# yandooo/cilium

Measured on AMD Instinct MI355X. Metric: L7 verdicts/sec + scanned GB/s (HBM roofline frac), 1/2/4/8 MI355X, higher is better.
Workload: dtype u8

## Files before the change

cilium_amd/csrc/kernels/kafka_classify.hip:

```cpp
#include <hip/hip_runtime.h>

#include "../device_tables.h"
#include "kafka_dec.h"
#include "launch.h"

namespace l7 {

namespace {

constexpr int kBlock = 256;


__device__ __forceinline__ uint32_t le_load4(Cur &c, const uint8_t *p) {
    const uintptr_t a = (uintptr_t)p;
    const uint32_t k = (uint32_t)(a & 15);
    if (k <= 12) {
        cur_fill(c, a);
        const uint32_t w0 = c.w0, w1 = c.w1, w2 = c.w2, w3 = c.w3;
        const uint32_t i = k >> 2;
        const uint32_t lo = i == 0 ? w0 : i == 1 ? w1 : i == 2 ? w2 : w3;
        const uint32_t hi = i == 0 ? w1 : i == 1 ? w2 : i == 2 ? w3 : 0u;
        return __builtin_amdgcn_alignbyte(hi, lo, k & 3);
    }
    uint32_t v = 0;
    for (int i = 0; i < 4; i++) v |= cur_byte(c, p + i) << (8 * i);
    return v;
}
__device__ __forceinline__ uint32_t bswap(uint32_t x) { return __builtin_amdgcn_perm(0, x, 0x00010203u); }

struct GRd {
    static constexpr bool kWin = true;
    const uint8_t *b;
    uintptr_t lastc;
    Cur cur;
    uint8_t *stage;
    uint32_t hlim;
    __device__ __forceinline__ void stage_head() {
        crc_stage(stage, reinterpret_cast<const uint8_t *>((uintptr_t)b & ~(uintptr_t)15), lastc);
        hlim = 64 - (uint32_t)((uintptr_t)b & 15);
    }
    __device__ __forceinline__ uint32_t slot_le4(uint32_t rel) {
        asm volatile("" : "+v"(rel));
        const uint32_t la = (uint32_t)(uintptr_t)(stage + 16 * lane_id());
        const uint32_t w0 = rel >> 2, w1 = w0 < 15 ? w0 + 1 : 15;
        uint32_t lo, hi;
        asm volatile("s_waitcnt vmcnt(0)\n\tds_read_b32 %0, %2\n\tds_read_b32 %1, %3\n\ts_waitcnt lgkmcnt(0)"
                     : "=&v"(lo), "=&v"(hi)
                     : "v"(la + ((w0 >> 2) << 10) + ((w0 & 3) << 2)), "v"(la + ((w1 >> 2) << 10) + ((w1 & 3) << 2))
                     : "memory");
        return __builtin_amdgcn_alignbyte(hi, lo, rel & 3);
    }
    __device__ __forceinline__ uint32_t le4(uint32_t pos) {
        if (pos + 4 <= hlim) return slot_le4(pos + (uint32_t)((uintptr_t)b & 15));
        return le_load4(cur, b + pos);
    }
    __device__ __forceinline__ uint64_t be(uint32_t pos, int n) {
        if (n <= 4 && pos + 4 <= hlim) {
            const uint32_t v = bswap(slot_le4(pos + (uint32_t)((uintptr_t)b & 15)));
            return n == 4 ? v : v >> (32 - 8 * n);
        }
        return be_load(cur, b + pos, n);
    }
    __device__ __forceinline__ void win9(uint32_t pos, uint32_t (&x)[9]) {
        const uintptr_t a = (uintptr_t)(b + pos);
        const uintptr_t c0 = a & ~(uintptr_t)15;
        uint32_t w[16];
        {
            hlim = 0;
            crc_stage(stage, reinterpret_cast<const uint8_t *>(c0), lastc);
            const uint32_t la = (uint32_t)(uintptr_t)(stage + 16 * lane_id());
            uint4 v0, v1, v2, v3;
            asm volatile("s_waitcnt vmcnt(0)\n\t"
                         "ds_read_b128 %0, %4\n\tds_read_b128 %1, %4 offset:1024\n\t"
                         "ds_read_b128 %2, %4 offset:2048\n\tds_read_b128 %3, %4 offset:3072\n\t"
                         "s_waitcnt lgkmcnt(0)"
                         : "=v"(v0), "=v"(v1), "=v"(v2), "=v"(v3)
                         : "v"(la)
                         : "memory");
            const uint4 vv[4] = {v0, v1, v2, v3};
#pragma unroll
            for (int k = 0; k < 4; k++) {
                w[4 * k] = vv[k].x; w[4 * k + 1] = vv[k].y; w[4 * k + 2] = vv[k].z; w[4 * k + 3] = vv[k].w;
            }
        }
        const uint32_t s = (uint32_t)(a & 15), q = s >> 2;
#pragma unroll
        for (int i = 0; i < 9; i++) {
            const uint32_t lo = q == 0 ? w[i] : q == 1 ? w[i + 1] : q == 2 ? w[i + 2] : w[i + 3];
            const uint32_t hi = q == 0 ? w[i + 1] : q == 1 ? w[i + 2] : q == 2 ? w[i + 3] : w[i + 4];
            x[i] = __builtin_amdgcn_alignbyte(hi, lo, s & 3);
        }
        cur.line = c0 + 16 <= lastc ? c0 + 16 : ~(uintptr_t)0;
        cur.w0 = w[4]; cur.w1 = w[5]; cur.w2 = w[6]; cur.w3 = w[7];
    }
    __device__ __forceinline__ uint32_t win_be4(uint32_t rel) { return bswap(slot_le4(rel)); }
};

template <class R>
struct KD {
    R *r;
    uint32_t pos, end;
    int32_t limit;
    int err;
};
template <class R>
__device__ __forceinline__ uint32_t kd_read(KD<R> &d, uint32_t n) {
    const uint32_t at = d.pos;
    if (n == 0) return at;
    uint32_t a = d.end - d.pos;
    if (d.limit >= 0 && (uint32_t)d.limit < a) a = (uint32_t)d.limit;
    if (a == 0) { d.err = 1; return at; }
    const uint32_t take = a < n ? a : n;
    d.pos += take;
    if (d.limit >= 0) d.limit -= (int32_t)take;
    if (take < n) d.err = 2;
    return at;
}
template <class R>
__device__ __forceinline__ int64_t kd_int(KD<R> &d, int n) {
    if (d.err) return 0;
    const uint32_t at = kd_read(d, (uint32_t)n);
    if (d.err) return 0;
    const uint64_t v = d.r->be(at, n);
    return n == 1 ? (int64_t)(int8_t)v : n == 2 ? (int64_t)(int16_t)v : n == 4 ? (int64_t)(int32_t)v : (int64_t)v;
}
template <class R>
__device__ __forceinline__ void kd_skip(KD<R> &d, int n) {
    if (d.err) return;
    kd_read(d, (uint32_t)n);
}
template <class R>
__device__ __forceinline__ void kd_string(KD<R> &d, uint32_t &off, uint32_t &len) {
    off = 0; len = 0;
    if (d.err) return;
    const int16_t sl = (int16_t)kd_int(d, 2);
    if (d.err || sl < 1) return;
    const uint32_t at = kd_read(d, (uint32_t)sl);
    if (d.err) return;
    off = at; len = (uint32_t)sl;
}
template <class R>
__device__ __forceinline__ int32_t kd_arraylen(KD<R> &d, bool nullable, bool &bad) {
    const int32_t l = (int32_t)kd_int(d, 4);
    bad = false;
    if (l < 0) { if (nullable) return -1; bad = true; return 0; }
    if ((uint32_t)l > kMaxParseBuf) { bad = true; return 0; }
    return l;
}
template <class R>
__device__ __forceinline__ bool kd_bulk(KD<R> &d, int32_t np, uint32_t esize) {
    if (d.err || np < 0) return false;
    uint32_t a = d.end - d.pos;
    if (d.limit >= 0 && (uint32_t)d.limit < a) a = (uint32_t)d.limit;
    const uint64_t need = (uint64_t)(uint32_t)np * esize;
    if (need > a) return false;
    d.pos += (uint32_t)need;
    if (d.limit >= 0) d.limit -= (int32_t)need;
    return true;
}
template <class R>
__device__ __forceinline__ void kd_bytes(KD<R> &d) {
    if (d.err) return;
    const int32_t sl = (int32_t)kd_int(d, 4);
    if (d.err || sl < 1) return;
    if ((uint32_t)sl > kMaxParseBuf) { d.err = 3; return; }
    kd_read(d, (uint32_t)sl);
}

template <class R, class H>
__device__ __forceinline__ int kd_message_set(R &r, uint32_t &pos, uint32_t end, int32_t size, int16_t version,
                                              bool &zflag, H &h) {
    if (size < 0) return 0;
    if ((uint32_t)size > kMaxParseBuf) return -1;
    KD<R> dec{&r, pos, end, size, 0};
    int rc = 0;
    if constexpr (R::kWin) {
        const uint32_t hmin = version >= 1 ? 22u : 14u;
        for (;;) {
            uint32_t avail = dec.end - dec.pos;
            if ((uint32_t)dec.limit < avail) avail = (uint32_t)dec.limit;
            if (avail < 12 + hmin) break;
            uint32_t x[9];
            r.win9(dec.pos, x);
            const uint32_t msize = bswap(x[2]);
            if ((int32_t)msize < (int32_t)hmin || 12 + msize > avail) break;
            const uint32_t at = dec.pos + 12;
            const uint32_t crc = bswap(x[3]);
            const uint32_t attr = (x[4] >> 8) & 0xFF;
            const int32_t klen = (int32_t)bswap(version >= 1 ? __builtin_amdgcn_alignbyte(x[7], x[6], 2)
                                                             : __builtin_amdgcn_alignbyte(x[5], x[4], 2));
            const uint32_t ko = at + (version >= 1 ? 14u : 6u);
            uint32_t vo = ko + 4;
            int32_t vlen;
            if (klen < 1) {
                vlen = (int32_t)bswap(version >= 1 ? __builtin_amdgcn_alignbyte(x[8], x[7], 2)
                                                   : __builtin_amdgcn_alignbyte(x[6], x[5], 2));
            } else {
                if ((uint32_t)klen > msize || vo + (uint32_t)klen + 4 > at + msize) break;
                vo += (uint32_t)klen;
                const uint32_t rel = vo - dec.pos + (uint32_t)((uintptr_t)(r.b + dec.pos) & 15);
                if (rel + 4 <= 64) {
                    vlen = (int32_t)r.win_be4(rel);
                } else {
                    const Cur keep = r.cur;
                    vlen = (int32_t)r.be(vo, 4);
                    r.cur = keep;
                }
            }
            if (vlen >= 1 && ((uint32_t)vlen > msize || vo + 4 + (uint32_t)vlen > at + msize)) break;
            dec.pos = at + msize;
            dec.limit -= (int32_t)(12 + msize);
            if (!h.msg_win(at + 4, msize - 4, crc)) { pos = dec.pos; return 0; }
            if ((attr & 3) == 3) { pos = dec.pos; return 0; }
            if (attr & 3) zflag = true;
        }
    }
    for (;;) {
        kd_skip(dec, 8);
        if (dec.err) break;
        const int32_t msize = (int32_t)kd_int(dec, 4);
        if (dec.err || msize <= 0) break;
        if ((uint32_t)msize > kMaxParseBuf) { rc = -1; break; }
        const uint32_t at = kd_read(dec, (uint32_t)msize);
        if (dec.err) break;
        KD<R> md{&r, at, at + (uint32_t)msize, -1, 0};
        const uint32_t crc = (uint32_t)kd_int(md, 4);
        if (msize <= 4) break;
        if (!h.msg(at + 4, (uint32_t)msize - 4, crc)) break;
        kd_skip(md, 1);
        const int8_t attr = (int8_t)kd_int(md, 1);
        if (version >= 1) kd_skip(md, 8);
        const int codec = attr & 3;
        if (codec == 3) break;
        kd_bytes(md);
        kd_bytes(md);
        if (md.err) { rc = -1; break; }
        if (codec != 0) zflag = true;
    }
    pos = dec.pos;
    return rc;
}

__device__ __forceinline__ bool is_topic_api_key(int k) {
    if (k < 0 || k > 37) return false;
    const uint64_t m = (1ull << 0) | (1ull << 1) | (1ull << 2) | (1ull << 3) | (1ull << 4) | (1ull << 5) | (1ull << 6) |
                       (1ull << 8) | (1ull << 9) | (1ull << 19) | (1ull << 20) | (1ull << 21) | (1ull << 23) |
                       (1ull << 24) | (1ull << 27) | (1ull << 28) | (1ull << 34) | (1ull << 35) | (1ull << 37);
    return (m >> k) & 1;
}
__device__ __forceinline__ int kind_typed(int kind) {
    return (kind == 0 || kind == 1 || kind == 2 || kind == 3 || kind == 8 || kind == 9) ? 1 : (kind == 10 ? 2 : 0);
}

template <class R, class H>
__device__ __forceinline__ int kafka_walk(R &r, uint32_t rawlen, int kind, bool &zflag, H &h) {
    KD<R> d{&r, 0, rawlen, -1, 0};
    bool bad = false;
    int rc = 0;
    kd_skip(d, 4); kd_skip(d, 2);
    const int16_t ver = (int16_t)kd_int(d, 2);
    kd_skip(d, 4);
    uint32_t co, cl;
    kd_string(d, co, cl);
    if (!d.err && cl > 0) h.client(co, cl);
    int32_t nt, np;
    uint32_t o, l;
    switch (kind) {
    case 0:
        if (ver >= 3) kd_string(d, o, l);
        kd_skip(d, 2); kd_skip(d, 4);
        nt = kd_arraylen(d, false, bad);
        if (bad) { rc = -1; break; }
        for (int32_t t = 0; t < nt && rc == 0; t++) {
            kd_string(d, o, l);
            if (d.err) break;
            h.topic(o, l);
            np = kd_arraylen(d, false, bad);
            if (bad) { rc = -1; break; }
            for (int32_t p = 0; p < np; p++) {
                kd_skip(d, 4);
                if (d.err) { rc = -1; break; }
                const int32_t ss = (int32_t)kd_int(d, 4);
                if (d.err) { rc = -1; break; }
                rc = kd_message_set(r, d.pos, d.end, ss, ver, zflag, h);
                if (rc) break;
            }
        }
        break;
    case 1:
        kd_skip(d, 4); kd_skip(d, 4); kd_skip(d, 4);
        if (ver >= 3) kd_skip(d, 4);
        if (ver >= 4) kd_skip(d, 1);
        nt = kd_arraylen(d, false, bad);
        if (bad) { rc = -1; break; }
        for (int32_t t = 0; t < nt && !d.err; t++) {
            kd_string(d, o, l);
            h.topic(o, l);
            np = kd_arraylen(d, false, bad);
            if (bad) { rc = -1; break; }
            if (kd_bulk(d, np, ver >= 5 ? 24u : 16u)) continue;
            for (int32_t p = 0; p < np && !d.err; p++) {
                kd_skip(d, 4); kd_skip(d, 8);
                if (ver >= 5) kd_skip(d, 8);
                kd_skip(d, 4);
            }
        }
        break;
    case 2:
        kd_skip(d, 4);
        if (ver >= 2) kd_skip(d, 1);
        nt = kd_arraylen(d, false, bad);
        if (bad) { rc = -1; break; }
        for (int32_t t = 0; t < nt && !d.err; t++) {
            kd_string(d, o, l);
            h.topic(o, l);
            np = kd_arraylen(d, false, bad);
            if (bad) { rc = -1; break; }
            if (kd_bulk(d, np, ver == 0 ? 16u : 12u)) continue;
            for (int32_t p = 0; p < np && !d.err; p++) {
                kd_skip(d, 4); kd_skip(d, 8);
                if (ver == 0) kd_skip(d, 4);
            }
        }
        break;
    case 3:
        nt = kd_arraylen(d, true, bad);
        if (bad) { rc = -1; break; }
        for (int32_t t = 0; t < nt && !d.err; t++) {
            kd_string(d, o, l);
            if (!d.err) h.topic(o, l);
        }
        if (ver >= 4) kd_skip(d, 1);
        break;
    case 8:
        kd_string(d, o, l);
        if (ver >= 1) { kd_skip(d, 4); kd_string(d, o, l); }
        if (ver >= 2) kd_skip(d, 8);
        nt = kd_arraylen(d, false, bad);
        if (bad) { rc = -1; break; }
        for (int32_t t = 0; t < nt && !d.err; t++) {
            kd_string(d, o, l);
            h.topic(o, l);
            np = kd_arraylen(d, false, bad);
            if (bad) { rc = -1; break; }
            for (int32_t p = 0; p < np && !d.err; p++) {
                kd_skip(d, 4); kd_skip(d, 8);
                if (ver == 1) kd_skip(d, 8);
                uint32_t o2, l2;
                kd_string(d, o2, l2);
            }
        }
        break;
    case 9:
        kd_string(d, o, l);
        nt = kd_arraylen(d, true, bad);
        if (bad) { rc = -1; break; }
        for (int32_t t = 0; t < nt && !d.err; t++) {
            kd_string(d, o, l);
            h.topic(o, l);
            np = kd_arraylen(d, false, bad);
            if (bad) { rc = -1; break; }
            if (kd_bulk(d, np, 4u)) continue;
            for (int32_t p = 0; p < np && !d.err; p++) kd_skip(d, 4);
        }
        break;
    case 10:
        kd_string(d, o, l);
        if (ver >= 1) kd_skip(d, 1);
        break;
    }
    if (rc == 0 && d.err) rc = -1;
    return rc;
}

template <class R>
__device__ __forceinline__ int32_t str_lookup(const DevStrSlot *tab, uint32_t mask, const uint8_t *strings, R &r,
                                              uint32_t pos, uint32_t n) {
    uint32_t h = kWHashSeed;
    uint32_t p0 = 0, p1 = 0, p2 = 0, p3 = 0;
    for (uint32_t i = 0; i < n; i += 4) {
        const uint32_t rem = n - i;
        const uint32_t keep = rem >= 4 ? 0xFFFFFFFFu : (1u << (8 * rem)) - 1u;
        const uint32_t w = r.le4(pos + i) & keep;
        h = l7_whash_step(h, w);
        p0 = i == 0 ? w : p0;
        p1 = i == 4 ? w : p1;
        p2 = i == 8 ? w : p2;
        p3 = i == 12 ? w : p3;
    }
    h = l7_whash_final(h, n);
    for (uint32_t slot = h & mask;; slot = (slot + 1) & mask) {
        const DevStrSlot e = tab[slot];
        if (!e.used) return -1;
        if (e.hash == h && e.len == n) {
            bool eq = e.pre[0] == p0 && e.pre[1] == p1 && e.pre[2] == p2 && e.pre[3] == p3;
            const uint32_t *t = reinterpret_cast<const uint32_t *>(strings + e.str_off);
            for (uint32_t i = 16; i < n && eq; i += 4) {
                const uint32_t rem = n - i;
                const uint32_t keep = rem >= 4 ? 0xFFFFFFFFu : (1u << (8 * rem)) - 1u;
                eq = t[i >> 2] == (r.le4(pos + i) & keep);
            }
            if (eq) return e.id;
        }
    }
}

struct ReqInfo {
    uint32_t kv;
    int32_t client;
    __device__ __forceinline__ int kind_() const { return (int)(int16_t)(kv >> 16); }
    __device__ __forceinline__ int version_() const { return (int)(int16_t)(kv & 0xFFFF); }
    __device__ __forceinline__ int typed_() const { return kind_typed(kind_()); }
};

__device__ __forceinline__ bool rule_matches(const DevKafkaRule &r, const ReqInfo &q) {
    if (!r.any_key && (q.kind_() < 0 || q.kind_() > 63 || !((r.keymask >> q.kind_()) & 1))) return false;
    if (r.has_version && r.version != q.version_()) return false;
    if (!r.has_topic && r.client < 0) return true;
    if (q.typed_() == 1) return r.client < 0 || r.client == q.client;
    if (q.typed_() == 2) return true;
    return !(r.has_topic && is_topic_api_key(q.kind_()));
}

__device__ __forceinline__ uint32_t topic_first(const KafkaTables &T, const DevKafkaRuleset &rs, const ReqInfo &q,
                                                int32_t tid) {
    if (tid < 0 || rs.ntopics == 0) return kInf;
    uint32_t off, cnt;
    if (rs.tdense_off != ~0u) {
        const uint4 *ep = reinterpret_cast<const uint4 *>(T.index + rs.tdense_off +
                                                          (uint32_t)(sizeof(DevKafkaTopicEnt) / 4) * (uint32_t)tid);
        const uint4 e0 = ep[0], e1 = ep[1], e2 = ep[2];
        off = e0.y;
        cnt = e0.z;
        if (cnt == 0) return kInf;
        DevKafkaRule r0;
        const uint32_t w[6] = {e1.x, e1.y, e1.z, e1.w, e2.x, e2.y};
        __builtin_memcpy(&r0, w, sizeof r0);
        if (rule_matches(r0, q)) return e0.x;
        for (uint32_t i = 1; i < cnt; i++) {
            const uint32_t p = T.index[off + i];
            if (rule_matches(T.rules[rs.rule_first + p], q)) return p;
        }
        return kInf;
    } else {
        const uint32_t *dir = T.index + rs.topics_off;
        uint32_t lo = 0, hi = rs.ntopics;
        while (lo < hi) {
            const uint32_t m = (lo + hi) >> 1;
            if (dir[3 * m] < (uint32_t)tid) lo = m + 1; else hi = m;
        }
        if (lo >= rs.ntopics || dir[3 * lo] != (uint32_t)tid) return kInf;
        off = dir[3 * lo + 1];
        cnt = dir[3 * lo + 2];
    }
    for (uint32_t i = 0; i < cnt; i++) {
        const uint32_t p = T.index[off + i];
        if (rule_matches(T.rules[rs.rule_first + p], q)) return p;
    }
    return kInf;
}

__device__ __forceinline__ uint32_t matches_rule(const KafkaTables &T, const DevKafkaRuleset &rs, const ReqInfo &q,
                                                 uint32_t ntopics, uint32_t cmax) {
    uint32_t best = kInf;
    if (ntopics == 0) {
        const int key = (q.kind_() >= 0 && q.kind_() < 64) ? q.kind_() : 64;
        const uint32_t off = T.index[rs.bykey_off + 2 * key], cnt = T.index[rs.bykey_off + 2 * key + 1];
        for (uint32_t i = 0; i < cnt; i++) {
            const uint32_t p = T.index[off + i];
            if (rule_matches(T.rules[rs.rule_first + p], q)) { best = p; break; }
        }
    } else {
        for (uint32_t i = 0; i < rs.ntopicless; i++) {
            const uint32_t p = T.index[rs.topicless_off + i];
            if (p >= cmax) break;
            if (rule_matches(T.rules[rs.rule_first + p], q)) { best = p; break; }
        }
        if (best == kInf) best = cmax;
    }
    return best;
}

struct NoTopicLog {};
struct TopicLog {
    LogSpan *row;
    uint32_t stride;
};
template <class L>
struct ExactHooks {
    const KafkaTables &T;
    const DevKafkaRuleset &rs;
    ReqInfo &q;
    GRd &r;
    const uint32_t *crctab;
    uint8_t *stage;
    uint32_t ntopics, cmax;
    L log;
    __device__ __forceinline__ void client(uint32_t o, uint32_t l) {
        q.client = str_lookup(T.client_hash, T.client_mask, T.strings, r, o, l);
        if (q.client < 0) q.client = -2;
    }
    __device__ __forceinline__ void topic(uint32_t o, uint32_t l) {
        if (q.typed_() != 1) return;
        if constexpr (!std::is_same<L, NoTopicLog>::value) {
            if (ntopics < log.stride) log.row[ntopics] = LogSpan{o, l};
        }
        ntopics++;
        const int32_t tid = l > 0 ? str_lookup(T.topic_hash, T.topic_mask, T.strings, r, o, l) : -1;
        const uint32_t e = topic_first(T, rs, q, tid);
        cmax = cmax > e ? cmax : e;
    }
    __device__ __forceinline__ bool msg(uint32_t pos, uint32_t n, uint32_t stored) {
        r.hlim = 0;
        return crc32_ieee_staged(crctab, r.cur, r.b + pos, n, stage, r.lastc) == stored;
    }
    __device__ __forceinline__ bool msg_win(uint32_t pos, uint32_t n, uint32_t stored) {
        return crc32_ieee_window(crctab, r.cur, r.b + pos, n, stage, r.lastc) == stored;
    }
};

}

template <int kWaves, bool kLog>
__global__ __launch_bounds__(kBlock) __attribute__((amdgpu_waves_per_eu(kWaves, 8))) void kafka_classify_kernel(
    Batch B, KafkaTables T, const uint32_t *__restrict__ sel, const uint32_t *__restrict__ sel_count,
    uint32_t answer_other, uint32_t *__restrict__ zlist, uint32_t *__restrict__ zcount, uint32_t *__restrict__ work,
    uint32_t main_sweep, LogRec *__restrict__ lrec, LogSpan *__restrict__ ltopics, uint32_t lstride) {
    const uint32_t n = B.n, nconns = B.nconns;
    static_assert(kBlock >= 256, "one CRC table entry per thread");
    __shared__ uint32_t crctab[kCrcTables * 256];
    __shared__ __attribute__((aligned(16))) uint8_t crcstage[kBlock / 64][4096];
    uint8_t *stage = crcstage[__builtin_amdgcn_readfirstlane((int)(threadIdx.x >> 6))];
    crc_tables_init(crctab, threadIdx.x);
    constexpr int kCls = L7_KAFKA_CLASSES;
    uint32_t kc[kCls] = {n};
    uint32_t m = n;
    if (sel) {
        m = 0;
        for (int c = 0; c < kCls; c++) { kc[c] = sel_count[c]; m += kc[c]; }
    }
    const uint32_t stride = main_sweep ? main_sweep : gridDim.x * kBlock;
    auto next_entry = [&](uint32_t i) -> uint32_t {
        if (!work) return i + stride;
        const uint32_t lane = lane_id();
        uint32_t t = 0;
        if (lane == (uint32_t)__builtin_amdgcn_readfirstlane(lane)) t = atomicAdd(work, 64u);
        return stride + __builtin_amdgcn_readfirstlane(t) + lane;
    };
    for (uint32_t i = main_sweep ? next_entry(0) : blockIdx.x * kBlock + threadIdx.x; i < m; i = next_entry(i)) {
        uint32_t idx = i;
        if (sel) {
            uint32_t c = 0, j = i;
            bool hit = false;
#pragma unroll
            for (int k = kCls - 1; k > 0; k--) {
                if (!hit) {
                    if (j >= kc[k]) j -= kc[k];
                    else { c = (uint32_t)k; hit = true; }
                }
            }
            idx = sel[(size_t)c * n + j];
        }
        const uint32_t ci = B.conn_ids[idx];
        const DevConn conn = ci < nconns ? B.conns[ci] : DevConn{-1, PROTO_NONE, 0, 0xFFFF};
        const uint64_t off = B.offs[idx];
        const uint32_t len = B.lens[idx];
        uint8_t verdict = V_PARSE_ERROR;
        int32_t rule = -1;
        uint32_t consumed = 0;
        bool zflag = false;
        if (conn.proto != PROTO_KAFKA || conn.ruleset < 0 || (uint32_t)conn.ruleset >= T.nrulesets) {
            if (!answer_other || (L7_PROTO_OWNED(conn.proto) && conn.proto != PROTO_KAFKA)) continue;
            verdict = V_UNSUPPORTED;
        }
        do {
            if (verdict == V_UNSUPPORTED) break;
            if (!l7_in_arena(off, len, B.arena_len)) { verdict = V_UNSUPPORTED; break; }
            if (len < 4) { verdict = V_INCOMPLETE; break; }
            GRd r{B.arena + off, ((uintptr_t)(B.arena + off) + len - 1) & ~(uintptr_t)15, {}, stage, 0};
            r.stage_head();
            r.cur.line = ~(uintptr_t)0;
            const int32_t size = (int32_t)r.be(0, 4);
            if (size <= 0) break;
            if (len < 6) { verdict = V_INCOMPLETE; break; }
            if ((uint64_t)(uint32_t)size + 4 > kMaxParseBuf) break;
            const uint32_t rawlen = (uint32_t)size + 4;
            if (rawlen > len) { verdict = V_INCOMPLETE; break; }
            if (rawlen < 12) break;
            ReqInfo q;
            q.kv = (uint32_t)r.be(4, 4);
            q.client = -2;
            const DevKafkaRuleset &rs = T.rulesets[conn.ruleset];
            using Log = typename std::conditional<kLog, TopicLog, NoTopicLog>::type;
            Log lg{};
            if constexpr (kLog) lg = TopicLog{ltopics + (size_t)idx * lstride, lstride};
            ExactHooks<Log> h{T, rs, q, r, crctab, stage, 0, 0, lg};
            if (q.typed_() && kafka_walk(r, rawlen, q.kind_(), zflag, h) == -1) break;
            consumed = rawlen;
            verdict = V_DENY;
            if constexpr (kLog) {
                const uint32_t corr = (uint32_t)r.be(8, 4);
                uint4 *o = reinterpret_cast<uint4 *>(lrec + idx);
                o[0] = make_uint4(LOG_KAFKA | (h.ntopics > lstride ? 0x100u : 0u) | (q.kv & 0xFFFF0000u),
                                  q.kv & 0xFFFFu, corr, h.ntopics);
                o[1] = make_uint4(0, 0, 0, 0);
            }
            if (!rs.any) break;
            const uint32_t best = matches_rule(T, rs, q, h.ntopics, h.cmax);
            if (best != kInf) { verdict = V_ALLOW; rule = T.rules[rs.rule_first + best].gid; }
        } while (false);
        B.verdict[idx] = verdict;
        B.rule[idx] = rule;
        B.consumed[idx] = consumed;
        if (zflag && zlist && (verdict == V_ALLOW || verdict == V_DENY)) zlist[atomicAdd(zcount, 1u)] = idx;
    }
}

hipError_t KafkaPhaseTimes(uint64_t *, bool) { return hipErrorNotSupported; }

hipError_t LaunchKafkaClassify(const Batch &B, const KafkaTables &T, const uint32_t *sel, const uint32_t *sel_count,
                               bool answer_other, uint32_t *zlist, uint32_t *zcount, uint32_t *work,
                               hipStream_t stream, int leave_per_cu, bool helper, const LogOut *log) {
    if (B.n == 0) return hipSuccess;
    uint32_t blocks = (B.n + kBlock - 1) / kBlock;
    const bool beside = leave_per_cu > 0;
    if (helper && (!beside || !work)) return hipErrorInvalidValue;
    const bool lg = log != nullptr;
    const auto kernel = lg ? kafka_classify_kernel<4, true>
                           : (beside ? kafka_classify_kernel<6, false> : kafka_classify_kernel<5, false>);
    static int cus[2][2] = {}, per_cu[2][2] = {};
    if (cus[lg][beside] == 0) {
        int dev = 0, c = 0, p = 0;
        if (hipGetDevice(&dev) == hipSuccess &&
            hipDeviceGetAttribute(&c, hipDeviceAttributeMultiprocessorCount, dev) == hipSuccess &&
            hipOccupancyMaxActiveBlocksPerMultiprocessor(&p, kernel, kBlock, 0) == hipSuccess && c > 0 && p > 0) {
            per_cu[lg][beside] = p;
            cus[lg][beside] = c;
        } else {
            per_cu[lg][beside] = 32;
            cus[lg][beside] = 256;
        }
    }
    const int pc = per_cu[lg][beside], ncu = cus[lg][beside];
    const int slots = beside && pc > leave_per_cu ? pc - leave_per_cu : pc;
    if (!work) blocks = blocks > 8192 ? 8192 : blocks;
    else if (blocks > (uint32_t)(ncu * slots)) blocks = (uint32_t)(ncu * slots);
    const uint32_t grid = helper ? min(blocks, (uint32_t)(ncu * min(leave_per_cu, pc))) : blocks;
    const uint32_t main_sweep = helper ? blocks * (uint32_t)kBlock : 0u;
    LogRec *lrec = lg ? log->rec : nullptr;
    LogSpan *ltopics = lg ? log->topics : nullptr;
    hipLaunchKernelGGL(kernel, dim3(grid), dim3(kBlock), 0, stream, B, T, sel, sel_count, answer_other ? 1u : 0u, zlist,
                       zcount, work, main_sweep, lrec, ltopics, lg ? log->stride : 0u);
    return hipGetLastError();
}

}
```

cilium_amd/csrc/kernels/kafka_dec.h:

```cpp
#pragma once
#include <hip/hip_runtime.h>

#include <stdint.h>

#include "gmem.h"

namespace l7 {
namespace {

constexpr uint32_t kMaxParseBuf = 6553500;
constexpr int kCrcSlices = 8;
constexpr int kCrcTables = 8;
__device__ __forceinline__ void crc_tables_init(uint32_t *tab, uint32_t t) {
    if (t < 256) {
        uint32_t c = t;
        for (int k = 0; k < 8; k++) c = (c & 1) ? 0xEDB88320u ^ (c >> 1) : c >> 1;
        tab[t] = c;
    }
    __syncthreads();
    if (t < 256) {
        uint32_t v = tab[t];
        for (int k = 1; k < kCrcTables; k++) {
            v = (v >> 8) ^ tab[v & 0xFF];
            tab[k * 256 + t] = v;
        }
    }
    __syncthreads();
}
__device__ __forceinline__ uint32_t crc_slice8(const uint32_t *tab, uint32_t lo, uint32_t hi) {
    return tab[7 * 256 + (lo & 0xFF)] ^ tab[6 * 256 + ((lo >> 8) & 0xFF)] ^ tab[5 * 256 + ((lo >> 16) & 0xFF)] ^
           tab[4 * 256 + (lo >> 24)] ^ tab[3 * 256 + (hi & 0xFF)] ^ tab[2 * 256 + ((hi >> 8) & 0xFF)] ^
           tab[1 * 256 + ((hi >> 16) & 0xFF)] ^ tab[hi >> 24];
}
constexpr uint32_t kInf = 0xFFFFFFFFu;
__device__ __forceinline__ uint32_t lane_id() {
    return __builtin_amdgcn_mbcnt_hi(~0u, __builtin_amdgcn_mbcnt_lo(~0u, 0u));
}

struct Cur {
    uintptr_t line;
    uint32_t w0, w1, w2, w3;
};
__device__ __forceinline__ void cur_fill(Cur &c, uintptr_t a) {
    const uintptr_t ln = a & ~(uintptr_t)15;
    if (ln != c.line) {
        const uint4 v = gload16(ln);
        c.w0 = v.x; c.w1 = v.y; c.w2 = v.z; c.w3 = v.w;
        c.line = ln;
    }
}
__device__ __forceinline__ uint32_t cur_word(const Cur &c, uint32_t k) {
    const uint32_t a = c.w0, b = c.w1, d = c.w2, e = c.w3;
    return k < 8 ? (k < 4 ? a : b) : (k < 12 ? d : e);
}
__device__ __forceinline__ uint32_t cur_byte(Cur &c, const uint8_t *p) {
    const uintptr_t a = (uintptr_t)p;
    cur_fill(c, a);
    const uint32_t k = (uint32_t)(a & 15);
    return (cur_word(c, k) >> ((k & 3) * 8)) & 0xFFu;
}

struct KDec {
    const uint8_t *b;
    uint32_t pos, end;
    int32_t limit;
    int err;
    Cur *c;
};

__device__ __forceinline__ uint32_t kavail(const KDec &d) {
    uint32_t a = d.end - d.pos;
    if (d.limit >= 0 && (uint32_t)d.limit < a) a = (uint32_t)d.limit;
    return a;
}
__device__ __forceinline__ uint32_t kread(KDec &d, uint32_t n) {
    uint32_t at = d.pos;
    if (n == 0) return at;
    uint32_t a = kavail(d);
    if (a == 0) { d.err = 1; return at; }
    uint32_t take = a < n ? a : n;
    d.pos += take;
    if (d.limit >= 0) d.limit -= (int32_t)take;
    if (take < n) d.err = 2;
    return at;
}
__device__ __forceinline__ uint32_t bswap32(uint32_t x) { return __builtin_amdgcn_perm(0, x, 0x00010203u); }
__device__ __forceinline__ uint64_t be_load(Cur &c, const uint8_t *p, int n) {
    const uintptr_t a = (uintptr_t)p;
    const uint32_t k = (uint32_t)(a & 15);
    if (n <= 4 && k + (uint32_t)n <= 16) {
        cur_fill(c, a);
        const uint32_t w0 = c.w0, w1 = c.w1, w2 = c.w2, w3 = c.w3;
        const uint32_t i = k >> 2;
        const uint32_t lo = i == 0 ? w0 : i == 1 ? w1 : i == 2 ? w2 : w3;
        const uint32_t hi = i == 0 ? w1 : i == 1 ? w2 : i == 2 ? w3 : 0u;
        const uint32_t v = bswap32(__builtin_amdgcn_alignbyte(hi, lo, k & 3));
        return n == 4 ? v : v >> (32 - 8 * n);
    }
    if (n == 8) return (be_load(c, p, 4) << 32) | be_load(c, p + 4, 4);
    uint64_t v = 0;
    for (int i = 0; i < n; i++) v = (v << 8) | cur_byte(c, p + i);
    return v;
}
__device__ __forceinline__ int64_t dec_int(KDec &d, int n) {
    if (d.err) return 0;
    uint32_t at = kread(d, (uint32_t)n);
    if (d.err) return 0;
    uint64_t v = be_load(*d.c, d.b + at, n);
    return n == 1 ? (int64_t)(int8_t)v : n == 2 ? (int64_t)(int16_t)v : n == 4 ? (int64_t)(int32_t)v : (int64_t)v;
}
__device__ __forceinline__ void dec_skip(KDec &d, int n) {
    if (d.err) return;
    kread(d, (uint32_t)n);
}
__device__ __forceinline__ void dec_string(KDec &d, uint32_t &off, uint32_t &len) {
    off = 0; len = 0;
    if (d.err) return;
    int16_t sl = (int16_t)dec_int(d, 2);
    if (d.err || sl < 1) return;
    uint32_t at = kread(d, (uint32_t)sl);
    if (d.err) return;
    off = at; len = (uint32_t)sl;
}
__device__ __forceinline__ int32_t dec_arraylen(KDec &d, bool nullable, bool &bad) {
    int32_t l = (int32_t)dec_int(d, 4);
    bad = false;
    if (l < 0) { if (nullable) return -1; bad = true; return 0; }
    if ((uint32_t)l > kMaxParseBuf) { bad = true; return 0; }
    return l;
}
__device__ __forceinline__ void dec_bytes(KDec &d) {
    if (d.err) return;
    int32_t sl = (int32_t)dec_int(d, 4);
    if (d.err || sl < 1) return;
    if ((uint32_t)sl > kMaxParseBuf) { d.err = 3; return; }
    kread(d, (uint32_t)sl);
}

__device__ __forceinline__ uint32_t crc32_ieee(const uint32_t *tab, Cur &cur, const uint8_t *p, uint32_t n) {
    uint32_t c = 0xFFFFFFFFu;
    uint32_t i = 0;
    for (; i < n && (((uintptr_t)(p + i)) & 15); i++) c = tab[(c ^ cur_byte(cur, p + i)) & 0xFF] ^ (c >> 8);
    for (; i + 64 <= n; i += 64) {
        const uint4 *q = reinterpret_cast<const uint4 *>(p + i);
        uint4 v[4];
#pragma unroll
        for (int j = 0; j < 4; j++) v[j] = q[j];
#pragma unroll
        for (int j = 0; j < 8; j++) {
            const uint4 &x = v[j >> 1];
            const uint32_t lo = ((j & 1) ? x.z : x.x) ^ c, hi = (j & 1) ? x.w : x.y;
            c = tab[7 * 256 + (lo & 0xFF)] ^ tab[6 * 256 + ((lo >> 8) & 0xFF)] ^ tab[5 * 256 + ((lo >> 16) & 0xFF)] ^
                tab[4 * 256 + (lo >> 24)] ^ tab[3 * 256 + (hi & 0xFF)] ^ tab[2 * 256 + ((hi >> 8) & 0xFF)] ^
                tab[1 * 256 + ((hi >> 16) & 0xFF)] ^ tab[hi >> 24];
        }
    }
    for (; i + 8 <= n; i += 8) {
        const uintptr_t a = (uintptr_t)(p + i);
        cur_fill(cur, a);
        const uint32_t k = (uint32_t)(a & 15);
        const uint32_t w0 = cur.w0, w1 = cur.w1, w2 = cur.w2, w3 = cur.w3;
        const uint32_t lo = (k ? w2 : w0) ^ c, hi = k ? w3 : w1;
        c = tab[7 * 256 + (lo & 0xFF)] ^ tab[6 * 256 + ((lo >> 8) & 0xFF)] ^ tab[5 * 256 + ((lo >> 16) & 0xFF)] ^
            tab[4 * 256 + (lo >> 24)] ^ tab[3 * 256 + (hi & 0xFF)] ^ tab[2 * 256 + ((hi >> 8) & 0xFF)] ^
            tab[1 * 256 + ((hi >> 16) & 0xFF)] ^ tab[hi >> 24];
    }
    for (; i < n; i++) c = tab[(c ^ cur_byte(cur, p + i)) & 0xFF] ^ (c >> 8);
    return ~c;
}


__device__ __forceinline__ uint32_t crc_step8(uint32_t tabaddr, uint32_t lo, uint32_t hi) {
    const uint32_t a0 = tabaddr + ((lo & 0xFF) << 2), a1 = tabaddr + (((lo >> 8) & 0xFF) << 2),
                   a2 = tabaddr + (((lo >> 16) & 0xFF) << 2), a3 = tabaddr + ((lo >> 24) << 2),
                   a4 = tabaddr + ((hi & 0xFF) << 2), a5 = tabaddr + (((hi >> 8) & 0xFF) << 2),
                   a6 = tabaddr + (((hi >> 16) & 0xFF) << 2), a7 = tabaddr + ((hi >> 24) << 2);
    uint32_t r0, r1, r2, r3, r4, r5, r6, r7;
    asm volatile(
        "ds_read_b32 %0, %8 offset:7168\n\tds_read_b32 %1, %9 offset:6144\n\t"
        "ds_read_b32 %2, %10 offset:5120\n\tds_read_b32 %3, %11 offset:4096\n\t"
        "ds_read_b32 %4, %12 offset:3072\n\tds_read_b32 %5, %13 offset:2048\n\t"
        "ds_read_b32 %6, %14 offset:1024\n\tds_read_b32 %7, %15\n\t"
        "s_waitcnt lgkmcnt(0)"
        : "=&v"(r0), "=&v"(r1), "=&v"(r2), "=&v"(r3), "=&v"(r4), "=&v"(r5), "=&v"(r6), "=&v"(r7)
        : "v"(a0), "v"(a1), "v"(a2), "v"(a3), "v"(a4), "v"(a5), "v"(a6), "v"(a7)
        : "memory");
    return (r0 ^ r1) ^ (r2 ^ r3) ^ (r4 ^ r5) ^ (r6 ^ r7);
}
__device__ __forceinline__ uint32_t crc_step4(uint32_t tabaddr, uint32_t x) {
    const uint32_t a0 = tabaddr + ((x & 0xFF) << 2), a1 = tabaddr + (((x >> 8) & 0xFF) << 2),
                   a2 = tabaddr + (((x >> 16) & 0xFF) << 2), a3 = tabaddr + ((x >> 24) << 2);
    uint32_t r0, r1, r2, r3;
    asm volatile(
        "ds_read_b32 %0, %4 offset:3072\n\tds_read_b32 %1, %5 offset:2048\n\t"
        "ds_read_b32 %2, %6 offset:1024\n\tds_read_b32 %3, %7\n\t"
        "s_waitcnt lgkmcnt(0)"
        : "=&v"(r0), "=&v"(r1), "=&v"(r2), "=&v"(r3)
        : "v"(a0), "v"(a1), "v"(a2), "v"(a3)
        : "memory");
    return (r0 ^ r1) ^ (r2 ^ r3);
}
__device__ __forceinline__ uint32_t crc_bytes3(uint32_t tabaddr, uint32_t c, uint32_t x, uint32_t r) {
    const uint32_t y = c ^ x;
    const uint32_t a0 = tabaddr + ((r - 1) << 10) + ((y & 0xFF) << 2);
    const uint32_t a1 = tabaddr + ((r - 2) << 10) + (((y >> 8) & 0xFF) << 2);
    const uint32_t a2 = tabaddr + (((y >> 16) & 0xFF) << 2);
    const uint32_t b0 = r >= 1 ? a0 : tabaddr, b1 = r >= 2 ? a1 : tabaddr, b2 = r >= 3 ? a2 : tabaddr;
    uint32_t r0, r1, r2;
    asm volatile("ds_read_b32 %0, %3\n\tds_read_b32 %1, %4\n\tds_read_b32 %2, %5\n\ts_waitcnt lgkmcnt(0)"
                 : "=&v"(r0), "=&v"(r1), "=&v"(r2)
                 : "v"(b0), "v"(b1), "v"(b2)
                 : "memory");
    return (c >> (8 * r)) ^ r0 ^ (r >= 2 ? r1 : 0u) ^ (r >= 3 ? r2 : 0u);
}
__device__ __forceinline__ uint32_t cur_word_at(const Cur &c, uint32_t k) {
    const uint32_t w0 = c.w0, w1 = c.w1, w2 = c.w2, w3 = c.w3;
    const uint32_t i = k >> 2;
    const uint32_t lo = i == 0 ? w0 : i == 1 ? w1 : i == 2 ? w2 : w3;
    const uint32_t hi = i == 0 ? w1 : i == 1 ? w2 : i == 2 ? w3 : 0u;
    return __builtin_amdgcn_alignbyte(hi, lo, k & 3);
}


__device__ __forceinline__ uint32_t crc_head(uint32_t tabaddr, Cur &cur, const uint8_t *p, uint32_t n, uint32_t &c) {
    uint32_t i = 0;
    const uint32_t k0 = (uint32_t)((uintptr_t)p & 15);
    uint32_t h = (16 - k0) & 15;
    if (h > n) h = n;
    if (h >= 4) {
        cur_fill(cur, (uintptr_t)p);
        if (h >= 8) {
            c = crc_step8(tabaddr, cur_word_at(cur, k0) ^ c, cur_word_at(cur, k0 + 4));
            i = 8;
        }
        if (h - i >= 4) {
            c = crc_step4(tabaddr, cur_word_at(cur, k0 + i) ^ c);
            i += 4;
        }
    }
    if (i < h) {
        cur_fill(cur, (uintptr_t)p);
        c = crc_bytes3(tabaddr, c, cur_word_at(cur, k0 + i), h - i);
        i = h;
    }
    return i;
}
__device__ __forceinline__ void crc_stage(uint8_t *stage, const uint8_t *q, uintptr_t lastc) {
#pragma unroll
    for (int k = 0; k < 4; k++) {
        const uintptr_t a = (uintptr_t)(q + 16 * k);
        __builtin_amdgcn_global_load_lds((const void *)(k == 0 || a <= lastc ? a : lastc),
                                         (__attribute__((address_space(3))) void *)(stage + k * 1024), 16, 0, 0);
    }
}
__device__ __forceinline__ uint32_t crc_batch(const uint32_t *tab, uint8_t *stage, uint32_t c, const uint8_t *next,
                                              uintptr_t lastc) {
    const uint32_t la = (uint32_t)(uintptr_t)(stage + 16 * lane_id());
    uint4 v0, v1, v2, v3;
    asm volatile("s_waitcnt vmcnt(0)\n\t"
                 "ds_read_b128 %0, %4\n\tds_read_b128 %1, %4 offset:1024\n\t"
                 "ds_read_b128 %2, %4 offset:2048\n\tds_read_b128 %3, %4 offset:3072\n\t"
                 "s_waitcnt lgkmcnt(0)"
                 : "=v"(v0), "=v"(v1), "=v"(v2), "=v"(v3)
                 : "v"(la)
                 : "memory");
    if (next) crc_stage(stage, next, lastc);
#pragma unroll
    for (int j = 0; j < 8; j++) {
        const uint4 x = j < 2 ? v0 : j < 4 ? v1 : j < 6 ? v2 : v3;
        const uint32_t lo = ((j & 1) ? x.z : x.x) ^ c, hi = (j & 1) ? x.w : x.y;
        c = crc_slice8(tab, lo, hi);
    }
    return c;
}
__device__ __forceinline__ uint32_t lds_word_at(uint32_t la, uint32_t j) {
    uint32_t x;
    asm volatile("ds_read_b32 %0, %1\n\ts_waitcnt lgkmcnt(0)" : "=v"(x) : "v"(la + ((j >> 4) << 10) + (j & 15)) : "memory");
    return x;
}
__device__ __forceinline__ uint32_t crc_last(uint32_t tabaddr, uint8_t *stage, uint32_t rem, uint32_t c,
                                             uint32_t j0 = 0) {
    const uint32_t la = (uint32_t)(uintptr_t)(stage + 16 * lane_id());
    asm volatile("s_waitcnt vmcnt(0)" ::: "memory");
    uint32_t j = j0;
    for (; j + 8 <= rem; j += 8) {
        uint64_t x;
        asm volatile("ds_read_b64 %0, %1\n\ts_waitcnt lgkmcnt(0)"
                     : "=v"(x)
                     : "v"(la + ((j >> 4) << 10) + (j & 8))
                     : "memory");
        c = crc_step8(tabaddr, (uint32_t)x ^ c, (uint32_t)(x >> 32));
    }
    if (j + 4 <= rem) {
        c = crc_step4(tabaddr, lds_word_at(la, j) ^ c);
        j += 4;
    }
    if (j < rem) c = crc_bytes3(tabaddr, c, lds_word_at(la, j), rem - j);
    return c;
}
__device__ __forceinline__ uint32_t crc32_ieee_staged(const uint32_t *tab, Cur &cur, const uint8_t *p, uint32_t n,
                                                      uint8_t *stage, uintptr_t lastc) {
    const uint32_t tabaddr = (uint32_t)(uintptr_t)tab;
    uint32_t c = 0xFFFFFFFFu;
    uint32_t i = crc_head(tabaddr, cur, p, n, c);
    if (i < n) {
        asm volatile("s_waitcnt vmcnt(0)" ::: "memory");
        crc_stage(stage, p + i, lastc);
        while (i + 64 <= n) {
            const bool more = i + 64 < n;
            c = crc_batch(tab, stage, c, more ? p + i + 64 : nullptr, lastc);
            i += 64;
        }
        if (i < n) c = crc_last(tabaddr, stage, n - i, c);
    }
    return ~c;
}
__device__ __forceinline__ uint32_t crc32_ieee_window(const uint32_t *tab, Cur &cur, const uint8_t *p, uint32_t n,
                                                      uint8_t *stage, uintptr_t lastc) {
    const uint32_t tabaddr = (uint32_t)(uintptr_t)tab;
    uint32_t c = 0xFFFFFFFFu;
    uint32_t i = crc_head(tabaddr, cur, p, n, c);
    if (i < n) {
        const uint8_t *c0 = reinterpret_cast<const uint8_t *>((uintptr_t)(p - 16) & ~(uintptr_t)15);
        const uint32_t o = (uint32_t)((p + i) - c0);
        if (n - i <= 64 - o) return ~crc_last(tabaddr, stage, o + (n - i), c, o);
        const uint32_t la = (uint32_t)(uintptr_t)(stage + 16 * lane_id());
        uint4 v1, v2, v3;
        asm volatile("ds_read_b128 %0, %3 offset:1024\n\tds_read_b128 %1, %3 offset:2048\n\t"
                     "ds_read_b128 %2, %3 offset:3072\n\ts_waitcnt lgkmcnt(0)"
                     : "=v"(v1), "=v"(v2), "=v"(v3)
                     : "v"(la)
                     : "memory");
        crc_stage(stage, c0 + 64, lastc);
        const uint32_t j0 = o == 16 ? 0 : 2;
#pragma unroll
        for (uint32_t j = 0; j < 6; j++) {
            if (j < j0) continue;
            const uint4 x = j < 2 ? v1 : j < 4 ? v2 : v3;
            const uint32_t lo = ((j & 1) ? x.z : x.x) ^ c, hi = (j & 1) ? x.w : x.y;
            c = crc_slice8(tab, lo, hi);
        }
        i += 64 - o;
        while (i + 64 <= n) {
            const bool more = i + 64 < n;
            c = crc_batch(tab, stage, c, more ? p + i + 64 : nullptr, lastc);
            i += 64;
        }
        if (i < n) c = crc_last(tabaddr, stage, n - i, c);
    }
    return ~c;
}

}
}
```

Baseline: 3.065 billion.

## Reuse staged LDS window across Kafka record header reads and CRC

Replaces absolute-address staging bookkeeping with a relative span base. The win9 header read now re-stages from global memory only when the 36-byte window falls outside the currently staged 64 bytes, and CRC over a record leaves the span pointing at the last staged block, so the next header can reuse it. This is meant to cut redundant global_load_lds transfers and the wait on them per record. It also shrinks per-lane state (32-bit end instead of pointers, a ruleset index instead of a reference) to ease register pressure, at the cost of more complex span arithmetic that could introduce stale-window bugs.

```diff
diff --git a/cilium_amd/csrc/kernels/kafka_classify.hip b/cilium_amd/csrc/kernels/kafka_classify.hip
--- a/cilium_amd/csrc/kernels/kafka_classify.hip
+++ b/cilium_amd/csrc/kernels/kafka_classify.hip
@@ -31,13 +31,23 @@
 struct GRd {
     static constexpr bool kWin = true;
     const uint8_t *b;
-    uintptr_t lastc;
+    uint32_t end;
+    __device__ __forceinline__ uint32_t lastr() const {
+        uint32_t e = end;
+        asm volatile("" : "+v"(e));
+        return (rel(e) - 1) & ~15u;
+    }
     Cur cur;
     uint8_t *stage;
-    uint32_t hlim;
+    uint32_t span;
+    __device__ __forceinline__ const uint8_t *base() const {
+        return reinterpret_cast<const uint8_t *>((uintptr_t)b & ~(uintptr_t)15);
+    }
+    __device__ __forceinline__ uintptr_t lastc() const { return (uintptr_t)base() + lastr(); }
+    __device__ __forceinline__ uint32_t rel(uint32_t pos) const { return pos + (uint32_t)((uintptr_t)b & 15); }
     __device__ __forceinline__ void stage_head() {
-        crc_stage(stage, reinterpret_cast<const uint8_t *>((uintptr_t)b & ~(uintptr_t)15), lastc);
-        hlim = 64 - (uint32_t)((uintptr_t)b & 15);
+        crc_stage_at(stage, base(), 0, lastr());
+        span = 0u - rel(0);
     }
     __device__ __forceinline__ uint32_t slot_le4(uint32_t rel) {
         asm volatile("" : "+v"(rel));
@@ -51,12 +61,14 @@
         return __builtin_amdgcn_alignbyte(hi, lo, rel & 3);
     }
     __device__ __forceinline__ uint32_t le4(uint32_t pos) {
-        if (pos + 4 <= hlim) return slot_le4(pos + (uint32_t)((uintptr_t)b & 15));
+        const uint32_t o = pos - span;
+        if (o <= 60u) return slot_le4(o);
         return le_load4(cur, b + pos);
     }
     __device__ __forceinline__ uint64_t be(uint32_t pos, int n) {
-        if (n <= 4 && pos + 4 <= hlim) {
-            const uint32_t v = bswap(slot_le4(pos + (uint32_t)((uintptr_t)b & 15)));
+        const uint32_t o = pos - span;
+        if (n <= 4 && o <= 60u) {
+            const uint32_t v = bswap(slot_le4(o));
             return n == 4 ? v : v >> (32 - 8 * n);
         }
         return be_load(cur, b + pos, n);
@@ -66,16 +78,21 @@
         const uintptr_t c0 = a & ~(uintptr_t)15;
         uint32_t w[16];
         {
-            hlim = 0;
-            crc_stage(stage, reinterpret_cast<const uint8_t *>(c0), lastc);
-            const uint32_t la = (uint32_t)(uintptr_t)(stage + 16 * lane_id());
+            const uint32_t s = rel(pos);
+            const uint32_t wb = ksched::window_base(span + rel(0), s);
+            if (wb - rel(0) != span) {
+                span = wb - rel(0);
+                crc_stage_at(stage, base(), wb, lastr());
+            }
+            const uint32_t la3 = (uint32_t)(uintptr_t)(stage + 16 * lane_id()) + 3072;
+            const uint32_t la = la3 - 3072 + (((s - wb) >> 4) << 10);
             uint4 v0, v1, v2, v3;
             asm volatile("s_waitcnt vmcnt(0)\n\t"
                          "ds_read_b128 %0, %4\n\tds_read_b128 %1, %4 offset:1024\n\t"
-                         "ds_read_b128 %2, %4 offset:2048\n\tds_read_b128 %3, %4 offset:3072\n\t"
+                         "ds_read_b128 %2, %4 offset:2048\n\tds_read_b128 %3, %5\n\t"
                          "s_waitcnt lgkmcnt(0)"
                          : "=v"(v0), "=v"(v1), "=v"(v2), "=v"(v3)
-                         : "v"(la)
+                         : "v"(la), "v"(la3)
                          : "memory");
             const uint4 vv[4] = {v0, v1, v2, v3};
 #pragma unroll
@@ -90,10 +107,10 @@
             const uint32_t hi = q == 0 ? w[i + 1] : q == 1 ? w[i + 2] : q == 2 ? w[i + 3] : w[i + 4];
             x[i] = __builtin_amdgcn_alignbyte(hi, lo, s & 3);
         }
-        cur.line = c0 + 16 <= lastc ? c0 + 16 : ~(uintptr_t)0;
+        cur.line = (rel(pos) & ~15u) + 16 <= lastr() ? c0 + 16 : ~(uintptr_t)0;
         cur.w0 = w[4]; cur.w1 = w[5]; cur.w2 = w[6]; cur.w3 = w[7];
     }
-    __device__ __forceinline__ uint32_t win_be4(uint32_t rel) { return bswap(slot_le4(rel)); }
+    __device__ __forceinline__ uint32_t win_be4(uint32_t o) { return bswap(slot_le4(o)); }
 };
 
 template <class R>
@@ -198,9 +215,9 @@
             } else {
                 if ((uint32_t)klen > msize || vo + (uint32_t)klen + 4 > at + msize) break;
                 vo += (uint32_t)klen;
-                const uint32_t rel = vo - dec.pos + (uint32_t)((uintptr_t)(r.b + dec.pos) & 15);
-                if (rel + 4 <= 64) {
-                    vlen = (int32_t)r.win_be4(rel);
+                const uint32_t o = vo - r.span;
+                if (o <= 60u) {
+                    vlen = (int32_t)r.win_be4(o);
                 } else {
                     const Cur keep = r.cur;
                     vlen = (int32_t)r.be(vo, 4);
@@ -271,13 +288,13 @@
         kd_skip(d, 2); kd_skip(d, 4);
         nt = kd_arraylen(d, false, bad);
         if (bad) { rc = -1; break; }
-        for (int32_t t = 0; t < nt && rc == 0; t++) {
+        for (; nt > 0 && rc == 0; nt--) {
             kd_string(d, o, l);
             if (d.err) break;
             h.topic(o, l);
             np = kd_arraylen(d, false, bad);
             if (bad) { rc = -1; break; }
-            for (int32_t p = 0; p < np; p++) {
+            for (; np > 0; np--) {
                 kd_skip(d, 4);
                 if (d.err) { rc = -1; break; }
                 const int32_t ss = (int32_t)kd_int(d, 4);
@@ -489,13 +506,18 @@
 template <class L>
 struct ExactHooks {
     const KafkaTables &T;
-    const DevKafkaRuleset &rs;
+    int32_t rsi;
     ReqInfo &q;
     GRd &r;
     const uint32_t *crctab;
     uint8_t *stage;
     uint32_t ntopics, cmax;
     L log;
+    __device__ __forceinline__ const DevKafkaRuleset &rs() const {
+        int32_t k = rsi;
+        asm volatile("" : "+v"(k));
+        return T.rulesets[k];
+    }
     __device__ __forceinline__ void client(uint32_t o, uint32_t l) {
         q.client = str_lookup(T.client_hash, T.client_mask, T.strings, r, o, l);
         if (q.client < 0) q.client = -2;
@@ -507,15 +529,17 @@
         }
         ntopics++;
         const int32_t tid = l > 0 ? str_lookup(T.topic_hash, T.topic_mask, T.strings, r, o, l) : -1;
-        const uint32_t e = topic_first(T, rs, q, tid);
+        const uint32_t e = topic_first(T, rs(), q, tid);
         cmax = cmax > e ? cmax : e;
     }
     __device__ __forceinline__ bool msg(uint32_t pos, uint32_t n, uint32_t stored) {
-        r.hlim = 0;
-        return crc32_ieee_staged(crctab, r.cur, r.b + pos, n, stage, r.lastc) == stored;
+        r.span = ksched::kNoSpan;
+        return crc32_ieee_staged(crctab, r.cur, r.b + pos, n, stage, r.lastc()) == stored;
     }
     __device__ __forceinline__ bool msg_win(uint32_t pos, uint32_t n, uint32_t stored) {
-        return crc32_ieee_window(crctab, r.cur, r.b + pos, n, stage, r.lastc) == stored;
+        const uint32_t p = r.rel(pos), wb = r.rel(r.span);
+        r.span = ksched::keep_base(wb, p + n) - r.rel(0);
+        return crc32_ieee_window(crctab, r.cur, r.b, wb, p, p + n, stage, r.lastr()) == stored;
     }
 };
 
@@ -577,7 +601,7 @@
             if (verdict == V_UNSUPPORTED) break;
             if (!l7_in_arena(off, len, B.arena_len)) { verdict = V_UNSUPPORTED; break; }
             if (len < 4) { verdict = V_INCOMPLETE; break; }
-            GRd r{B.arena + off, ((uintptr_t)(B.arena + off) + len - 1) & ~(uintptr_t)15, {}, stage, 0};
+            GRd r{B.arena + off, len, {}, stage, ksched::kNoSpan};
             r.stage_head();
             r.cur.line = ~(uintptr_t)0;
             const int32_t size = (int32_t)r.be(0, 4);
@@ -586,15 +610,15 @@
             if ((uint64_t)(uint32_t)size + 4 > kMaxParseBuf) break;
             const uint32_t rawlen = (uint32_t)size + 4;
             if (rawlen > len) { verdict = V_INCOMPLETE; break; }
+            r.end = rawlen;
             if (rawlen < 12) break;
             ReqInfo q;
             q.kv = (uint32_t)r.be(4, 4);
             q.client = -2;
-            const DevKafkaRuleset &rs = T.rulesets[conn.ruleset];
             using Log = typename std::conditional<kLog, TopicLog, NoTopicLog>::type;
             Log lg{};
             if constexpr (kLog) lg = TopicLog{ltopics + (size_t)idx * lstride, lstride};
-            ExactHooks<Log> h{T, rs, q, r, crctab, stage, 0, 0, lg};
+            ExactHooks<Log> h{T, conn.ruleset, q, r, crctab, stage, 0, 0, lg};
             if (q.typed_() && kafka_walk(r, rawlen, q.kind_(), zflag, h) == -1) break;
             consumed = rawlen;
             verdict = V_DENY;
@@ -605,6 +629,7 @@
                                   q.kv & 0xFFFFu, corr, h.ntopics);
                 o[1] = make_uint4(0, 0, 0, 0);
             }
+            const DevKafkaRuleset &rs = h.rs();
             if (!rs.any) break;
             const uint32_t best = matches_rule(T, rs, q, h.ntopics, h.cmax);
             if (best != kInf) { verdict = V_ALLOW; rule = T.rules[rs.rule_first + best].gid; }
diff --git a/cilium_amd/csrc/kernels/kafka_dec.h b/cilium_amd/csrc/kernels/kafka_dec.h
--- a/cilium_amd/csrc/kernels/kafka_dec.h
+++ b/cilium_amd/csrc/kernels/kafka_dec.h
@@ -4,6 +4,7 @@
 #include <stdint.h>
 
 #include "gmem.h"
+#include "kafka_sched.h"
 
 namespace l7 {
 namespace {
@@ -253,8 +254,17 @@
                                          (__attribute__((address_space(3))) void *)(stage + k * 1024), 16, 0, 0);
     }
 }
-__device__ __forceinline__ uint32_t crc_batch(const uint32_t *tab, uint8_t *stage, uint32_t c, const uint8_t *next,
-                                              uintptr_t lastc) {
+__device__ __forceinline__ void crc_stage_at(uint8_t *stage, const uint8_t *o, uint32_t x, uint32_t lastr) {
+    const uint32_t k0 = (uint32_t)((uintptr_t)o & 15);
+#pragma unroll
+    for (int k = 0; k < 4; k++) {
+        const uint32_t y = x + 16 * k <= lastr ? x + 16 * k : lastr;
+        __builtin_amdgcn_global_load_lds((const void *)(o + (y - k0)),
+                                         (__attribute__((address_space(3))) void *)(stage + k * 1024), 16, 0, 0);
+    }
+}
+template <class StageNext>
+__device__ __forceinline__ uint32_t crc_batch(const uint32_t *tab, uint8_t *stage, uint32_t c, StageNext stage_next) {
     const uint32_t la = (uint32_t)(uintptr_t)(stage + 16 * lane_id());
     uint4 v0, v1, v2, v3;
     asm volatile("s_waitcnt vmcnt(0)\n\t"
@@ -264,7 +274,7 @@
                  : "=v"(v0), "=v"(v1), "=v"(v2), "=v"(v3)
                  : "v"(la)
                  : "memory");
-    if (next) crc_stage(stage, next, lastc);
+    stage_next();
 #pragma unroll
     for (int j = 0; j < 8; j++) {
         const uint4 x = j < 2 ? v0 : j < 4 ? v1 : j < 6 ? v2 : v3;
@@ -308,22 +318,26 @@
         crc_stage(stage, p + i, lastc);
         while (i + 64 <= n) {
             const bool more = i + 64 < n;
-            c = crc_batch(tab, stage, c, more ? p + i + 64 : nullptr, lastc);
+            c = crc_batch(tab, stage, c, [&] { if (more) crc_stage(stage, p + i + 64, lastc); });
             i += 64;
         }
         if (i < n) c = crc_last(tabaddr, stage, n - i, c);
     }
     return ~c;
 }
-__device__ __forceinline__ uint32_t crc32_ieee_window(const uint32_t *tab, Cur &cur, const uint8_t *p, uint32_t n,
-                                                      uint8_t *stage, uintptr_t lastc) {
-    const uint32_t tabaddr = (uint32_t)(uintptr_t)tab;
-    uint32_t c = 0xFFFFFFFFu;
-    uint32_t i = crc_head(tabaddr, cur, p, n, c);
-    if (i < n) {
-        const uint8_t *c0 = reinterpret_cast<const uint8_t *>((uintptr_t)(p - 16) & ~(uintptr_t)15);
-        const uint32_t o = (uint32_t)((p + i) - c0);
-        if (n - i <= 64 - o) return ~crc_last(tabaddr, stage, o + (n - i), c, o);
+struct CrcWindowRun {
+    const uint32_t *tab;
+    Cur &cur;
+    const uint8_t *b;
+    uint8_t *stage;
+    uint32_t lastr;
+    uint32_t c;
+    __device__ __forceinline__ uint32_t tabaddr() const { return (uint32_t)(uintptr_t)tab; }
+    __device__ __forceinline__ void head(uint32_t p, uint32_t h) {
+        crc_head(tabaddr(), cur, b + (p - (uint32_t)((uintptr_t)b & 15)), h, c);
+    }
+    __device__ __forceinline__ void slot(uint32_t, uint32_t lo, uint32_t hi) { c = crc_last(tabaddr(), stage, hi, c, lo); }
+    __device__ __forceinline__ void window(uint32_t, uint32_t lo, uint32_t next) {
         const uint32_t la = (uint32_t)(uintptr_t)(stage + 16 * lane_id());
         uint4 v1, v2, v3;
         asm volatile("ds_read_b128 %0, %3 offset:1024\n\tds_read_b128 %1, %3 offset:2048\n\t"
@@ -331,25 +345,26 @@
                      : "=v"(v1), "=v"(v2), "=v"(v3)
                      : "v"(la)
                      : "memory");
-        crc_stage(stage, c0 + 64, lastc);
-        const uint32_t j0 = o == 16 ? 0 : 2;
+        crc_stage_at(stage, b, next, lastr);
+        const uint32_t j0 = (lo - 16) >> 3;
 #pragma unroll
         for (uint32_t j = 0; j < 6; j++) {
             if (j < j0) continue;
             const uint4 x = j < 2 ? v1 : j < 4 ? v2 : v3;
-            const uint32_t lo = ((j & 1) ? x.z : x.x) ^ c, hi = (j & 1) ? x.w : x.y;
-            c = crc_slice8(tab, lo, hi);
-        }
-        i += 64 - o;
-        while (i + 64 <= n) {
-            const bool more = i + 64 < n;
-            c = crc_batch(tab, stage, c, more ? p + i + 64 : nullptr, lastc);
-            i += 64;
-        }
-        if (i < n) c = crc_last(tabaddr, stage, n - i, c);
-    }
-    return ~c;
-}
-
-}
-}
+            const uint32_t lo_ = ((j & 1) ? x.z : x.x) ^ c, hi_ = (j & 1) ? x.w : x.y;
+            c = crc_slice8(tab, lo_, hi_);
+        }
+    }
+    __device__ __forceinline__ void block(uint32_t, uint32_t next) {
+        c = crc_batch(tab, stage, c, [&] { if (next != ksched::kNoSpan) crc_stage_at(stage, b, next, lastr); });
+    }
+};
+__device__ __forceinline__ uint32_t crc32_ieee_window(const uint32_t *tab, Cur &cur, const uint8_t *b, uint32_t wb,
+                                                      uint32_t p, uint32_t e, uint8_t *stage, uint32_t lastr) {
+    CrcWindowRun run{tab, cur, b, stage, lastr, 0xFFFFFFFFu};
+    ksched::crc_schedule(wb, p, e, run);
+    return ~run.c;
+}
+
+}
+}
diff --git a/cilium_amd/csrc/kernels/kafka_sched.h b/cilium_amd/csrc/kernels/kafka_sched.h
--- /dev/null
+++ b/cilium_amd/csrc/kernels/kafka_sched.h
@@ -0,0 +1,41 @@
+#pragma once
+#include <stdint.h>
+
+#if defined(__HIPCC__) || defined(__CUDACC__)
+#define L7_KSCHED_FN __host__ __device__ __forceinline__
+#else
+#define L7_KSCHED_FN inline
+#endif
+
+namespace l7 {
+namespace ksched {
+
+constexpr uint32_t kNoSpan = 0x80000000u;
+constexpr uint32_t kWindow = 36;
+
+L7_KSCHED_FN bool in_span(uint32_t sb, uint32_t pos, uint32_t n) { return pos - sb <= 64u - n; }
+L7_KSCHED_FN uint32_t window_base(uint32_t sb, uint32_t s) { return in_span(sb, s, kWindow) ? sb : s & ~15u; }
+L7_KSCHED_FN uint32_t keep_base(uint32_t wb, uint32_t e) { return wb + ((e - wb - 1u) & ~63u); }
+
+template <class V>
+L7_KSCHED_FN void crc_schedule(uint32_t wb, uint32_t p, uint32_t e, V &v) {
+    uint32_t h = (16u - (p & 15u)) & 15u;
+    if (h > e - p) h = e - p;
+    if (h) v.head(p, h);
+    const uint32_t i = p + h;
+    if (i >= e) return;
+    if (e <= wb + 64u) {
+        v.slot(wb, i - wb, e - wb);
+        return;
+    }
+    uint32_t a = wb + 64u;
+    v.window(wb, i - wb, a);
+    while (e - a >= 64u) {
+        v.block(a, e - a > 64u ? a + 64u : kNoSpan);
+        a += 64u;
+    }
+    if (a < e) v.slot(a, 0u, e - a);
+}
+
+}
+}
```

After: 3.099 billion (median of 6 runs). +1.1%, better.
